# hasindu2008/cornetto

Measured on AMD Instinct MI355X. Metric: Gbases/s scanned (telowin+sdust+boringbits), higher is better.
Workload: dtype u8/u16 integer

## Files before the change

### cornetto_amd/__init__.py

```python
import ctypes as C
import os

import numpy as np

__all__ = ["lib", "Accel", "AccelError", "HIT_DT", "WIN_DT", "IVL_DT", "TELROW_DT", "khash_str_order", "panel_boring", "REG_DT", "REGREC_DT", "build",
           "LIB_PATH", "CLI_PATH"]

HERE = os.path.dirname(os.path.abspath(__file__))
DEV_LIB_PATH = os.path.join(HERE, "libcornetto_hip_dev.so")
LIB_PATH = os.environ.get("CORNETTO_LIB") or os.path.join(HERE, "libcornetto_hip.so")
CLI_PATH = os.path.join(HERE, "cornetto")

HIT_DT = np.dtype([("ctg", "<i4"), ("strand", "<i4"), ("start", "<i4"), ("end", "<i4")])
WIN_DT = np.dtype([("ctg", "<i4"), ("start", "<i4"), ("end", "<i4"), ("car", "<i4")])
IVL_DT = np.dtype([("ctg", "<i4"), ("start", "<i4"), ("finish", "<i4")])
TELROW_DT = np.dtype([("ctg", "<i4"), ("start", "<i4"), ("end", "<i4"), ("matched", "<i4")])
FQREC_DT = np.dtype([("head", "<i8"), ("seq", "<i8"), ("qual", "<i8"), ("len", "<i4"), ("name_len", "<i4"),
                     ("comment_len", "<i4"), ("keep", "<i4")])
EMITREC_DT = np.dtype([("ctg", "<i4"), ("rc", "<i4"), ("head", "<i8"), ("head_len", "<i8")])
FAREC_DT = np.dtype([("head", "<i8"), ("len", "<i8"), ("name_len", "<i4"), ("pad", "<i4")])
REG_DT = np.dtype([("st", "<i4"), ("end", "<i4"), ("depth", "<i4"), ("mq_depth", "<i4")])
REGREC_DT = np.dtype([("ctg", "<i4"), ("st", "<i4"), ("end", "<i4"), ("depth", "<i4"), ("mq_depth", "<i4")])
REGPK_DT = np.dtype([("st", "<i4"), ("depth", "<u2"), ("mq_depth", "<u2")])

# ... 342 lines not shown

    def telofind(self, asm, motif=b"TTAGGG"):
        p, n = C.c_void_p(), C.c_int64()
        self._chk(self.L.cornetto_telofind(self.h, asm.ptr, motif, C.byref(p), C.byref(n)))
        return _take(self.L, p, n.value, HIT_DT)

    def telowin_threshold(self, thr, identity):
        return self.L.cornetto_telowin_threshold(thr, identity)

    def telowin(self, hits, ctg_len, thr_adj):
        hits = np.ascontiguousarray(hits, dtype=HIT_DT)
        ctg_len = np.ascontiguousarray(ctg_len, dtype=np.int32)
        p, n = C.c_void_p(), C.c_int64()
        self._chk(self.L.cornetto_telowin(self.h, hits.ctypes.data, hits.size, ctg_len.ctypes.data, ctg_len.size,
                                          thr_adj, C.byref(p), C.byref(n)))
        return _take(self.L, p, n.value, WIN_DT)

    def telo_scan(self, asm, motif, thr_adj, want_hits=True):
        ph, nh, pw, nw = C.c_void_p(), C.c_int64(), C.c_void_p(), C.c_int64()
        self._chk(self.L.cornetto_telo_scan(self.h, asm.ptr, motif, thr_adj,
                                            C.byref(ph) if want_hits else None, C.byref(nh) if want_hits else None,
                                            C.byref(pw), C.byref(nw)))
        hits = _take(self.L, ph, nh.value, HIT_DT) if want_hits else None
        return hits, _take(self.L, pw, nw.value, WIN_DT)

    def telo_ends(self, asm, motif, thr_adj, merge_dist=100, ends=50000):
        p, n = C.c_void_p(), C.c_int64()
        self._chk(self.L.cornetto_telo_ends(self.h, asm.ptr, motif, thr_adj, merge_dist, ends, C.byref(p), C.byref(n)))
        return _take(self.L, p, n.value, IVL_DT)

    def sdust(self, asm, T=20, W=64):
        p, n = C.c_void_p(), C.c_int64()
        self._chk(self.L.cornetto_sdust_asm(self.h, asm.ptr, T, W, C.byref(p), C.byref(n)))
        return _take(self.L, p, n.value, IVL_DT)

    def sdust_begin(self, asm, T=20, W=64):
        self._chk(self.L.cornetto_sdust_asm_begin(self.h, asm.ptr, T, W))

    def sdust_end(self, asm, T=20, W=64):
        p, n = C.c_void_p(), C.c_int64()
        self._chk(self.L.cornetto_sdust_asm_end(self.h, asm.ptr, T, W, C.byref(p), C.byref(n)))
        return _take(self.L, p, n.value, IVL_DT)

    def sdust_stats(self, asm, T=20, W=64):
        self.L.cornetto_accel_sdust_stats(self.h, 1, None, 0)
        try:
            self.sdust(asm, T, W)
        finally:
            out = np.zeros(256, dtype=np.uint64)
            n = self.L.cornetto_accel_sdust_stats(self.h, 0, out.ctypes.data, 256)
        s = [int(x) for x in out[:n]]
        waves = s[254]
        if n > 207 and s[206]:
            return {"kernel": "sd_sift", "chunks": s[255], "tiles_of_64_bases": s[206], "positions_ct_above_T10": s[203], "after_L1": s[204], "after_L2": s[205],
                    "resolve_steps": s[200], "resolve_window_reads": s[201], "dp_tiles": s[208], "passes_with_candidates": s[202], "base_by_base_steps_of_chunks_with_other_bytes": s[207],
                    "window_reads_behind_a_gap_of": {"2": s[209], "3-4": s[210], "5-8": s[211]} if n > 211 else None}
        if not waves or not s[2]:
            return None
        hist = []
        for b in range(32):
            w = s[16 + 4 * b]
            if w:
                hist.append({"ms": [b * 0.5, b * 0.5 + 0.5], "waves": w, "jobs": s[18 + 4 * b], "find_perfect": s[19 + 4 * b], "find_perfect_with_candidates": s[17 + 4 * b]})
        return {"waves": waves, "chunks": s[255], "chunks_sampled_low_complexity": s[7], "wave_steps": s[2], "find_perfect_calls": s[3],
                "find_perfect_with_candidates": s[10], "plain_groups": s[4], "wave_ms_avg": round(s[5] / waves / 1e5, 3), "wave_ms_max": round(s[6] / 1e5, 3),
                "queue_fetch_rounds_per_wave": round(s[11] / waves, 1), "wave_time_histogram": hist}

    def cov_select_merged(self, cov, lo, hi, low_mq, edge_len, min_ctg_len, boring, merge_dist=1000, min_len=30000):
        p, n = C.c_void_p(), C.c_int64()
        self._chk(self.L.cornetto_cov_select_merged(self.h, cov.ptr, lo, hi, low_mq, edge_len, min_ctg_len, 1 if boring else 0, merge_dist, min_len,
                                                    C.byref(p), C.byref(n)))
        return _take(self.L, p, n.value, IVL_DT)

    def ivl_merge(self, ivls, dist):
        ivls = np.ascontiguousarray(ivls, dtype=IVL_DT)
        p, n = C.c_void_p(), C.c_int64()
        self._chk(self.L.cornetto_ivl_merge(self.h, ivls.ctypes.data, len(ivls), dist, C.byref(p), C.byref(n)))
        return _take(self.L, p, n.value, IVL_DT)

    def telobreaks(self, ctg_len, sd, tel):
        ctg_len = np.ascontiguousarray(ctg_len, dtype=np.int32)
        sd = np.ascontiguousarray(sd, dtype=IVL_DT)
        tel = np.ascontiguousarray(tel, dtype=TELROW_DT)
        p, n = C.c_void_p(), C.c_int64()
        self._chk(self.L.cornetto_telobreaks(self.h, ctg_len.ctypes.data, len(ctg_len), sd.ctypes.data, len(sd), tel.ctypes.data, len(tel),
                                             C.byref(p), C.byref(n)))
        return _take(self.L, p, n.value, IVL_DT)

    def cov_upload(self, depths, mqs):
        d = [np.ascontiguousarray(x, dtype=np.uint16) for x in depths]
        q = [np.ascontiguousarray(x, dtype=np.uint16) for x in mqs]
        n = len(d)
        pd = (C.c_void_p * max(n, 1))(*[a.ctypes.data for a in d])
        pq = (C.c_void_p * max(n, 1))(*[a.ctypes.data for a in q])
        lens = np.array([a.size for a in d], dtype=np.int32)
        out = C.c_void_p()
        self._chk(self.L.cornetto_cov_upload(self.h, pd, pq, lens.ctypes.data, n, C.byref(out)))
        return _Resident(self, out, self.L.cornetto_cov_free, lens)

    def cov_wrap(self, d_depth, d_mq, offsets, lens):
        offsets = np.ascontiguousarray(offsets, dtype=np.int64)
        lens = np.ascontiguousarray(lens, dtype=np.int32)
        out = C.c_void_p()
        self._chk(self.L.cornetto_cov_wrap(self.h, d_depth, d_mq, offsets.ctypes.data, lens.ctypes.data, len(lens), C.byref(out)))
        return _Resident(self, out, self.L.cornetto_cov_free, lens)

    def cov_shard(self, src_acc, cov, ctgs):
# ... 181 lines not shown
```

### cornetto_amd/csrc/sdust.hip

```cpp
#include <algorithm>
#include <type_traits>
#include <ctime>
#include <sched.h>

#include "common.hpp"
#include "scan.hpp"
#include "tiles.hpp"
#include "ivlmerge.hpp"

namespace {

__device__ __forceinline__ int nt4_code(uint32_t c);
struct SdArgs;
struct SdChunk;
template <bool LEAN = false>
__device__ int sd_find_start(const SdArgs &A, const SdChunk ch, const uint8_t *seq);

struct SdChunk {
    int32_t ctg, start, end;
};
struct SdChunkFill {
    SdChunk *out;
    const int32_t *len;
    int32_t chunk;
// ... 1554 lines not shown
        unsigned long long *d_tot = (unsigned long long *)cn_ws(h, WS_SD_STATS, 2048 + 64 * 64);
        unsigned long long *p_tot = (unsigned long long *)cn_pin(h, PIN_SMALL, 2048);
        if (!d_cnt || !d_tot || !p_tot) return cn_fail(h, CORNETTO_E_NOMEM, "sdust: workspace allocation failed");
        uint32_t *d_off = d_cnt + nc;
        stamp("small workspaces");
        const bool env_stats = CN_DEV_INT("CORNETTO_SDUST_STATS", 0) != 0;
        const bool want_stats = env_stats || h->sd_stats != 0;
        size_t cap = (size_t)std::max<int64_t>(16, chunk / 32);
        cap = (size_t)CN_DEV_INT("CORNETTO_SDUST_CAP", (int)cap);
        if (h->dev[WS_SD_OUT].bytes / (nc * sizeof(uint2)) > cap) cap = h->dev[WS_SD_OUT].bytes / (nc * sizeof(uint2));
        unsigned long long tot = 0;
        uint2 *d_out = nullptr;
        const int64_t est_key = key * 131 + T * 1031 + W;
        const bool one_go = w64_path && sift_on && !want_stats && a->sd_est_key == est_key && a->sd_est_rows >= 0 && CN_DEV_INT("CORNETTO_SDUST_FUSED", 1);
        if (phase == 1 && !one_go)
            return CORNETTO_OK;
        for (int attempt = 0; attempt < 4; ++attempt) {
            d_out = (uint2 *)cn_ws(h, WS_SD_OUT, nc * cap * sizeof(uint2));
            if (!d_out) return cn_fail(h, CORNETTO_E_NOMEM, "sdust: workspace allocation of %zu bytes failed", nc * cap * sizeof(uint2));
            CN_HIP(h, hipMemsetAsync(d_tot, 0, 2048 + 64 * 64, h->stream));
            uint32_t *d_slots = (uint32_t *)cn_ws(h, WS_SD_OFF, (size_t)(std::max<int64_t>(sd_waves, 1) + SD_WPB) * 64 * 64 * sizeof(uint32_t));
            if (!d_slots) return cn_fail(h, CORNETTO_E_NOMEM, "sdust: workspace allocation failed");
            stamp("row + slot workspaces");
            const bool use_w64 = w64_path;
            SdArgs A{a->d_bases, a->d_off, a->d_len, d_chunks, (int32_t)nc, T, W, d_out, d_cnt, (uint32_t)cap,
                     want_stats ? d_tot + 2 : nullptr, reinterpret_cast<uint32_t *>(d_tot + 1), d_slots, nullptr,
                     reinterpret_cast<uint32_t *>(d_tot + 8), nullptr, 0, CN_DEV_INT("CORNETTO_SDUST_RUNON", 1), (int32_t)chunk, a->d_wtab, a->d_wtab_base, reinterpret_cast<uint32_t *>(d_tot + 1) + 1};
            unsigned nb = (unsigned)((nc + 63) / 64);
            bool sift_walk_pending = false;
            bool dense_pending = false;
            struct DenseJoin {
                cornetto_accel_t *h;
                bool *pending;
                ~DenseJoin() { if (*pending && h->stream2) (void)hipStreamSynchronize(h->stream2); }
            } dense_join{h, &dense_pending};
            if (use_w64 && sift_on) {
                CN_HIP(h, hipMemsetAsync(d_cnt, 0, nc * 4, h->stream));
                const uint32_t reg_cap = (uint32_t)(chunk + 128);
                const uint32_t lds_wave = sift_lds_bytes(reg_cap);
                int lmin = 1;
                while (5 * (lmin + 1) <= T && lmin < 16) ++lmin;
                const bool walk_known = a->d_sd_walk && a->sd_walk_key == key;
                const size_t walk_words = 2 + 4 * nc + 2;
                if (!walk_known) {
                    if (a->d_sd_walk) { (void)hipFree(a->d_sd_walk); a->d_sd_walk = nullptr; }
                    a->sd_walk_key = -1;
                    if (cn_obj_malloc(h, (void **)&a->d_sd_walk, walk_words * 4) != hipSuccess) return cn_fail(h, CORNETTO_E_NOMEM, "sdust: device allocation failed");
                    CN_HIP(h, hipMemsetAsync(a->d_sd_walk, 0, (2 + 2 * nc) * 4, h->stream));
                }
                uint32_t *d_wflag = a->d_sd_walk + 2 + nc, *d_wrank = d_wflag + nc, *d_worder = d_wrank + nc;
                SiftArgs S{a->d_bases, a->d_off, a->d_len, d_chunks, (int32_t)nc, T, W, lds_wave, reg_cap,
                           walk_known ? d_worder : nullptr, walk_known ? nullptr : a->d_sd_walk, walk_known ? nullptr : d_wflag,
                           reinterpret_cast<uint32_t *>(d_tot + 256), T / 10 + 1, lmin, CN_DEV_INT("CORNETTO_SIFT_ABL", 0),
                           std::min(65, std::max(1, CN_DEV_INT("CORNETTO_SIFT_DP", 24))), std::min(65, std::max(1, CN_DEV_INT("CORNETTO_SIFT_L2SKIP", 48)))};
                sift_walk_pending = !walk_known;
                SdArgs R = A;
                R.stats = want_stats ? d_tot + 200 : nullptr;
                const bool cap_default = reg_cap == SIFT_CAP_DEFAULT && !CN_DEV_INT("CORNETTO_SIFT_GENERIC", 0) && !CN_DEV_INT("CORNETTO_SIFT_ABL", 0);
                if (h->sift_per_cu == 0 || h->sift_per_cu_default != (cap_default ? 1 : 0)) {
                    int per_cu = 0;
                    const hipError_t oe = cap_default ? hipOccupancyMaxActiveBlocksPerMultiprocessor(&per_cu, sd_sift<false, SIFT_CAP_DEFAULT>, 64 * SIFT_WPB, lds_wave * SIFT_WPB)
                                                      : hipOccupancyMaxActiveBlocksPerMultiprocessor(&per_cu, sd_sift<false>, 64 * SIFT_WPB, lds_wave * SIFT_WPB);
                    if (oe != hipSuccess || per_cu < 1) per_cu = 8;
                    h->sift_per_cu = per_cu;
                    h->sift_per_cu_default = cap_default ? 1 : 0;
                }
                const int per_cu_all = std::max(1, std::min<int>(h->sift_per_cu, (int)(163840 / ((lds_wave * SIFT_WPB + 1279) / 1280 * 1280))));
                const bool free_now = __atomic_load_n(&h->boost, __ATOMIC_ACQUIRE) != 0;
                const size_t cus_n = (size_t)std::max(h->sd_cus, 1);
                const size_t slots_all = (size_t)per_cu_all * cus_n;
                const size_t slots = free_now ? slots_all : std::max<size_t>(cus_n, slots_all * (size_t)h->share / 100);
                const size_t all_blocks = (nc + SIFT_WPB - 1) / SIFT_WPB;
                const unsigned nbk = (unsigned)std::min<size_t>(all_blocks, (size_t)CN_DEV_INT("CORNETTO_SIFT_BLOCKS", (int)slots));
                const unsigned extra = (unsigned)std::min<size_t>(all_blocks > nbk ? all_blocks - nbk : 0, slots_all > slots ? slots_all - slots : 0);
                const bool may_help = phase == 0 && extra > 0 && !want_stats && h->share < CN_DEV_INT("CORNETTO_SDUST_HELP_BELOW", 70);
                if (may_help) {
                    if (!h->stream2) {
                        int pr_least = 0, pr_greatest = 0;
                        (void)hipDeviceGetStreamPriorityRange(&pr_least, &pr_greatest);
                        CN_HIP(h, hipStreamCreateWithPriority(&h->stream2, hipStreamNonBlocking, pr_greatest));
                        CN_HIP(h, hipEventCreateWithFlags(&h->ev2, hipEventDisableTiming));
                        CN_HIP(h, hipEventCreateWithFlags(&h->ev1, hipEventDisableTiming));
                    }
                    if (!h->ev3) CN_HIP(h, hipEventCreateWithFlags(&h->ev3, hipEventDisableTiming));
                    CN_HIP(h, hipEventRecord(h->ev1, h->stream));
                }
                stamp("set up");
                if (want_stats) CN_LAUNCH(h, "sdust_kernel", sd_sift<true><<<dim3(nbk), dim3(64 * SIFT_WPB), lds_wave * SIFT_WPB, h->stream>>>(S, R));
                else if (cap_default) CN_LAUNCH(h, "sdust_kernel", sd_sift<false, SIFT_CAP_DEFAULT><<<dim3(nbk), dim3(64 * SIFT_WPB), lds_wave * SIFT_WPB, h->stream>>>(S, R));
                else CN_LAUNCH(h, "sdust_kernel", sd_sift<false><<<dim3(nbk), dim3(64 * SIFT_WPB), lds_wave * SIFT_WPB, h->stream>>>(S, R));
                __atomic_fetch_add(&h->launch_seq, 1ull, __ATOMIC_RELEASE);
                if (may_help) {
                    CN_HIP(h, hipEventRecord(h->ev3, h->stream));
                    bool helped = false;
                    while (hipEventQuery(h->ev3) == hipErrorNotReady) {
                        if (!helped && __atomic_load_n(&h->boost, __ATOMIC_ACQUIRE) != 0) {
                            CN_HIP(h, hipStreamWaitEvent(h->stream2, h->ev1, 0));
                            if (cap_default) sd_sift<false, SIFT_CAP_DEFAULT><<<dim3(extra), dim3(64 * SIFT_WPB), lds_wave * SIFT_WPB, h->stream2>>>(S, R);
                            else sd_sift<false><<<dim3(extra), dim3(64 * SIFT_WPB), lds_wave * SIFT_WPB, h->stream2>>>(S, R);
                            dense_pending = true;
                            CN_HIP(h, hipGetLastError());
                            CN_HIP(h, hipEventRecord(h->ev2, h->stream2));
                            helped = true;
                        }
                        sched_yield();
                    }
                    if (helped) CN_HIP(h, hipStreamWaitEvent(h->stream, h->ev2, 0));
// ... 118 lines not shown
                dense_pending = false;
            }
            CN_TRY(cnscan::exclusive_u32(h, "sdust_scan", d_cnt, (int64_t)nc, 1, d_off, d_tot));
            if (one_go) {
                size_t n_cap = (size_t)(a->sd_est_rows + a->sd_est_rows / 8 + 4096);
                if (CN_DEV_INT("CORNETTO_SDUST_EST_FORCE", 0) > 0) n_cap = (size_t)CN_DEV_INT("CORNETTO_SDUST_EST_FORCE", 0);
                const size_t m_cap = (size_t)(a->sd_est_out + a->sd_est_out / 16 + 1024);
                uint8_t *ws = (uint8_t *)cn_ws(h, WS_SD_DST, 2 * n_cap * sizeof(cornetto_ivl_t) + cnivl::ws_bytes(n_cap));
                cornetto_ivl_t *of = (cornetto_ivl_t *)cn_result_alloc(std::max<size_t>(m_cap * sizeof(cornetto_ivl_t), (size_t)1 << 20));
                if (ws && of && n_cap < 0x7fffffffull) {
                    cornetto_ivl_t *d_dst = (cornetto_ivl_t *)(ws + cnivl::ws_bytes(n_cap)), *d_st = d_dst + n_cap;
                    const unsigned nbg = (unsigned)((nc + 255) / 256);
                    CN_LAUNCH(h, "sdust_gather", sdust_gather<<<dim3(nbg), dim3(256), 0, h->stream>>>(d_out, d_cnt, d_off, (uint32_t)cap, d_chunks, (int32_t)nc, d_dst, (uint32_t)n_cap));
                    CN_HIP(h, hipMemsetAsync(d_tot + 9, 0xFF, 8, h->stream));
                    int rcf = cnivl::merge_fused(h, "sdust_stitch", d_dst, d_tot, (int64_t)n_cap, 0, d_st, d_tot + 9);
                    if (rcf != CORNETTO_OK) { cornetto_free(of); return rcf; }
                    stamp("tail queued");
                    if (hipMemcpyAsync(of, d_st, m_cap * sizeof(cornetto_ivl_t), hipMemcpyDeviceToHost, h->stream) != hipSuccess ||
                        hipMemcpyAsync(p_tot, d_tot, 128, hipMemcpyDeviceToHost, h->stream) != hipSuccess) {
                        (void)hipStreamSynchronize(h->stream);
                        cornetto_free(of);
                        return cn_fail(h, CORNETTO_E_HIP, "sdust: stitch / copy back failed");
                    }
                    if (phase == 1) {
                        h->sd_pend.state = 1; h->sd_pend.a = a; h->sd_pend.T = T; h->sd_pend.W = W; h->sd_pend.of = of;
                        h->sd_pend.m_cap = m_cap; h->sd_pend.n_cap = n_cap; h->sd_pend.cap = cap; h->sd_pend.key = key; h->sd_pend.walk_pending = sift_walk_pending;
                        return CORNETTO_OK;
                    }
                    const int fin = sd_one_go_finish(h, a, of, p_tot, cap, n_cap, m_cap, key, sift_walk_pending, ivls, n_ivls);
                    if (fin <= 0) {
                        if (fin == 0) stamp("results on the host (one go)");
                        return fin;
                    }
                } else if (of) {
                    cornetto_free(of);
                }
            }
            stamp("main kernel queued");
            CN_HIP(h, hipMemcpyAsync(p_tot, d_tot, want_stats ? 2048 : 128, hipMemcpyDeviceToHost, h->stream));
            CN_HIP(h, hipStreamSynchronize(h->stream));
            stamp("main kernel done");
            if (want_stats) {
                memcpy(h->sd_last, p_tot, 2048);
                if (a->sd_flagged >= 0) h->sd_last[7] = (unsigned long long)a->sd_flagged;
                h->sd_last[254] = nb;
                h->sd_last[255] = nc;
            }
            if (env_stats)
                for (int b = 0; b < 32; ++b)
                    if (p_tot[16 + 4 * b])
                        fprintf(stderr, "[sdust stats]   waves that ran %4.1f-%4.1f ms: %6llu, job fetches %llu, find_perfect calls %llu (%llu with candidates)\n", b * 0.5, b * 0.5 + 0.5,
                                p_tot[16 + 4 * b], p_tot[18 + 4 * b], p_tot[19 + 4 * b], p_tot[17 + 4 * b]);
            if (env_stats && sift_on)
                fprintf(stderr, "[sdust stats] sift: tiles %llu, positions with ct > T/10 %llu, after L1 %llu, after L2 %llu; resolve: steps %llu, window reads %llu (behind a gap of 2 / 3-4 / 5-8: %llu / %llu / %llu), dp tiles %llu; passes with candidates %llu; base-by-base steps of chunks with other bytes %llu\n",
                        p_tot[206], p_tot[203], p_tot[204], p_tot[205], p_tot[200], p_tot[201], p_tot[209], p_tot[210], p_tot[211], p_tot[208], p_tot[202], p_tot[207]);
            if (env_stats)
                fprintf(stderr, "[sdust stats] flagged low-complexity %llu; chunks %zu waves %u wave-steps %llu find_perfect calls %llu (%llu with candidates) plain groups %llu; wave time avg %.1f us max %.1f us; queue: %.1f fetch rounds and %.1f us per wave\n", p_tot[7], nc, nb,
                        p_tot[2], p_tot[3], p_tot[10], p_tot[4], nb ? (double)p_tot[5] / nb / 100.0 : 0.0, (double)p_tot[6] / 100.0, nb ? (double)p_tot[11] / nb : 0.0, nb ? (double)p_tot[12] / nb / 100.0 : 0.0);
            const uint32_t ovf = (uint32_t)(p_tot[1] & 0xFFFFFFFFull);
            const bool need_wtab = (p_tot[1] >> 32) != 0;
            if (need_wtab) {
                if (a->d_wtab) return cn_fail(h, CORNETTO_E_HIP, "sdust: word-count table requested twice");
                std::vector<int64_t> base(a->n + 1, 0);
                for (int32_t c = 0; c < a->n; ++c) base[c + 1] = base[c] + a->len[c] / SD_WBLK + 2;
                a->n_wblocks = base[a->n];
                uint32_t *d_wcnt = nullptr;
                if (hipMalloc((void **)&a->d_wtab, ((size_t)a->n_wblocks + 1) * 4) != hipSuccess ||
                    hipMalloc((void **)&a->d_wtab_base, ((size_t)a->n + 1) * 8) != hipSuccess ||
                    hipMalloc((void **)&d_wcnt, ((size_t)a->n_wblocks + 1) * 4) != hipSuccess)
                    return cn_fail(h, CORNETTO_E_NOMEM, "sdust: word-count table allocation failed");
                CN_HIP(h, hipMemcpyAsync(a->d_wtab_base, base.data(), ((size_t)a->n + 1) * 8, hipMemcpyHostToDevice, h->stream));
                const unsigned nbw = (unsigned)((a->n_wblocks + 255) / 256);
                CN_LAUNCH(h, "sd_wordcount", sd_wordcount<<<dim3(nbw), dim3(256), 0, h->stream>>>(a->d_bases, a->d_off, a->d_len, a->d_wtab_base, a->n,
                                                                                         a->n_wblocks, d_wcnt));
                int rc = cnscan::exclusive_u32(h, "sd_wordscan", d_wcnt, a->n_wblocks, 1, a->d_wtab, nullptr);
                hipError_t e = hipStreamSynchronize(h->stream);
                (void)hipFree(d_wcnt);
                if (rc != CORNETTO_OK) return rc;
                if (e != hipSuccess) return cn_fail(h, CORNETTO_E_HIP, "sdust: word-count table build failed");
                continue;
            }
            if (sift_walk_pending && !need_wtab) a->sd_walk_key = key;
            if (ovf <= cap) {
                tot = p_tot[0];
                break;
            }
            if (attempt >= 2) return cn_fail(h, CORNETTO_E_HIP, "sdust: a chunk produced %u intervals after resizing to %zu", ovf, cap);
            cap = ovf;
        }
        if (tot > 0x7fffffffull) return cn_fail(h, CORNETTO_E_UNSUPPORTED, "sdust: %llu intervals", tot);
        o = (cornetto_ivl_t *)cn_result_alloc((tot ? tot : 1) * sizeof(cornetto_ivl_t));
        if (!o) return cn_fail(h, CORNETTO_E_NOMEM, "sdust: host allocation failed");
        stamp("result buffer");
        if (tot > 0) {
            const size_t n = (size_t)tot;
            uint8_t *ws = (uint8_t *)cn_ws(h, WS_SD_DST, 2 * n * sizeof(cornetto_ivl_t) + cnivl::ws_bytes(n));
            if (!ws) { cornetto_free(o); return cn_fail(h, CORNETTO_E_NOMEM, "sdust: workspace allocation failed"); }
            cornetto_ivl_t *d_dst = (cornetto_ivl_t *)(ws + cnivl::ws_bytes(n)), *d_st = d_dst + n;
            const unsigned nbg = (unsigned)((nc + 255) / 256);
            CN_LAUNCH(h, "sdust_gather", sdust_gather<<<dim3(nbg), dim3(256), 0, h->stream>>>(d_out, d_cnt, d_off, (uint32_t)cap, d_chunks, (int32_t)nc, d_dst));
            CN_TRY(cnivl::merge(h, "sdust_stitch", d_dst, (int64_t)n, 0, ws, d_st, d_tot + 9));
            stamp("gather+stitch queued");
            if (trace) { (void)hipStreamSynchronize(h->stream); stamp("gather+stitch done (trace only)"); }
            if (hipMemcpyAsync(o, d_st, n * sizeof(cornetto_ivl_t), hipMemcpyDeviceToHost, h->stream) != hipSuccess ||
                hipMemcpyAsync(p_tot, d_tot + 9, 8, hipMemcpyDeviceToHost, h->stream) != hipSuccess ||
                hipStreamSynchronize(h->stream) != hipSuccess) {
                cornetto_free(o);
// ... 148 lines not shown
```

### cornetto_amd/csrc/sdust_sift.hpp

```cpp
#pragma once

struct SiftArgs {
    const uint8_t *bases;
    const int64_t *ctg_off;
    const int32_t *ctg_len;
    const SdChunk *chunks;
    int32_t n_chunks;
    int32_t T, W;
    uint32_t lds_per_wave;
    uint32_t reg_cap;
    const uint32_t *order;
    uint32_t *walk_out;
    uint32_t *iswalk_out;
    uint32_t *counter;
    int32_t thr, lmin;
    int32_t abl;
    int32_t dp_min;
    int32_t l2_skip;
};

#ifndef SIFT_WPB
#define SIFT_WPB 1
#endif
constexpr int SIFT_NCTR = 64;
constexpr int SIFT_PAD = 16;
#ifndef SIFT_K
#define SIFT_K 16
#endif
constexpr int SIFT_LS = SIFT_K - 1;
constexpr int SIFT_FIXED = 1024 + 512;
__host__ __device__ constexpr uint32_t sift_lds_bytes(uint32_t cap) { return (SIFT_FIXED + cap / 4 + 2 * (SIFT_PAD + cap) + 16 + 15) / 16 * 16; }


__device__ __forceinline__ uint32_t sd_codes4(uint32_t word)
{
    const uint32_t y = word & 0xDFDFDFDFu, idx = y & 0x07070707u;
    const uint32_t code = __builtin_amdgcn_perm(0x02000003u, 0x01000000u, idx);
    const uint32_t d = y ^ __builtin_amdgcn_perm(0x47FFFF54u, 0x43FF41FFu, idx);
    const uint32_t nz = ((d & 0x7F7F7F7Fu) + 0x7F7F7F7Fu) | d;
    return code | ((nz >> 5) & 0x04040404u);
}
__device__ __forceinline__ uint32_t sd_words4(uint32_t cn, uint32_t pcn)
{
    const uint32_t y1 = __builtin_amdgcn_alignbyte(cn, pcn, 3);
    const uint32_t y2 = __builtin_amdgcn_alignbyte(cn, pcn, 2);
    const uint32_t t = (cn & 0x03030303u) | ((y1 & 0x03030303u) << 2) | ((y2 & 0x03030303u) << 4);
    return t | (((cn | y1 | y2) & 0x04040404u) << 4);
}

__device__ __forceinline__ int sd_mbcnt64(unsigned long long m)
{
    return (int)__builtin_amdgcn_mbcnt_hi((uint32_t)(m >> 32), __builtin_amdgcn_mbcnt_lo((uint32_t)m, 0u));
}
__device__ __forceinline__ int sd_dpp_shr1(int old, int src, bool zero_fill)
{
    return zero_fill ? __builtin_amdgcn_update_dpp(0, src, 0x138, 0xF, 0xF, true) : __builtin_amdgcn_update_dpp(old, src, 0x138, 0xF, 0xF, false);
}

__device__ const uint32_t sd_recip_tab[64] = {0x0u, 0x0u, 0x80000000u, 0x55555556u, 0x40000000u, 0x33333334u, 0x2AAAAAABu, 0x24924925u, 0x20000000u, 0x1C71C71Du, 0x1999999Au, 0x1745D175u, 0x15555556u, 0x13B13B14u, 0x12492493u, 0x11111112u, 0x10000000u, 0xF0F0F10u, 0xE38E38Fu, 0xD79435Fu, 0xCCCCCCDu, 0xC30C30Du, 0xBA2E8BBu, 0xB21642Du, 0xAAAAAABu, 0xA3D70A4u, 0x9D89D8Au, 0x97B425Fu, 0x924924Au, 0x8D3DCB1u, 0x8888889u, 0x8421085u, 0x8000000u, 0x7C1F07Du, 0x7878788u, 0x7507508u, 0x71C71C8u, 0x6EB3E46u, 0x6BCA1B0u, 0x6906907u, 0x6666667u, 0x63E7064u, 0x6186187u, 0x5F417D1u, 0x5D1745Eu, 0x5B05B06u, 0x590B217u, 0x572620Bu, 0x5555556u, 0x539782Au, 0x51EB852u, 0x5050506u, 0x4EC4EC5u, 0x4D4873Fu, 0x4BDA130u, 0x4A7904Bu, 0x4924925u, 0x47DC120u, 0x469EE59u, 0x456C798u, 0x4444445u, 0x4325C54u, 0x4210843u, 0x4104105u};

__device__ __forceinline__ uint32_t sd_scan_max_dpp(uint32_t x)
{
    asm volatile("s_nop 1\n\t"
                 "v_max_u32_dpp %0, %0, %0 row_shr:1 row_mask:0xf bank_mask:0xf\n\ts_nop 1\n\t"
                 "v_max_u32_dpp %0, %0, %0 row_shr:2 row_mask:0xf bank_mask:0xf\n\ts_nop 1\n\t"
                 "v_max_u32_dpp %0, %0, %0 row_shr:4 row_mask:0xf bank_mask:0xf\n\ts_nop 1\n\t"
                 "v_max_u32_dpp %0, %0, %0 row_shr:8 row_mask:0xf bank_mask:0xf\n\ts_nop 1\n\t"
                 "v_max_u32_dpp %0, %0, %0 row_bcast:15 row_mask:0xa bank_mask:0xf\n\ts_nop 1\n\t"
                 "v_max_u32_dpp %0, %0, %0 row_bcast:31 row_mask:0xc bank_mask:0xf\n\ts_nop 1"
                 : "+v"(x));
    return x;
}

__device__ __forceinline__ int sd_wave_find_start(const SdChunk ch, const uint8_t *seq, int W, int lane)
{
    if (ch.start <= 0) return 0;
    const int y = ch.start - 2 * W;
    if (y <= 2) return 0;
    int need = W - 2;
    for (int tile = (y - 1) >> 6, it = 0; tile >= 0 && it < 64; --tile, ++it) {
        const int p = tile * 64 + lane;
        const bool isb = p < y && nt4_code(seq[p]) < 4;
        const unsigned long long b = sd_ballot(isb);
        need -= __popcll(b & (b << 1) & (b << 2));
        if (need <= 0 || tile == 0) return tile * 64;
    }
    return -2;
}

#ifndef SIFT_CHUNK_DEFAULT
#define SIFT_CHUNK_DEFAULT 1792
#endif
constexpr uint32_t SIFT_CAP_DEFAULT = SIFT_CHUNK_DEFAULT + 128;
template <bool STATS, uint32_t CAP = 0>
__global__ __launch_bounds__(64 * SIFT_WPB) __attribute__((amdgpu_waves_per_eu(CAP ? 7 : 6))) void sd_sift(SiftArgs A, SdArgs O)
{
    extern __shared__ __attribute__((aligned(16))) uint8_t sift_lds[];
    const int lane = threadIdx.x & 63;
    const int wave = SIFT_WPB == 1 ? 0 : __builtin_amdgcn_readfirstlane((int)(threadIdx.x >> 6));
    uint8_t *const L = sift_lds + (size_t)wave * (CAP ? sift_lds_bytes(CAP) : A.lds_per_wave);
    uint32_t *const tab = reinterpret_cast<uint32_t *>(L);
    uint16_t *const tl = reinterpret_cast<uint16_t *>(L + 1024);
    uint16_t *const tl2 = tl + 128;
    uint32_t *const sb = reinterpret_cast<uint32_t *>(L + SIFT_FIXED);
    const uint32_t cap = CAP ? CAP : A.reg_cap;
#ifdef CN_DEV
    const int abl = CAP ? 0 : A.abl;
#else
    constexpr int abl = 0;
#endif
    constexpr int STAGE_ROUNDS = CAP ? (int)((CAP + 1023) / 1024) : 4;
    uint32_t *const cb = sb + (cap >> 5);
    uint4 *const col = reinterpret_cast<uint4 *>(tab);
    uint8_t *const wc = L + SIFT_FIXED + cap / 4 + 2 * SIFT_PAD;
    const int T = A.T, W = A.W, CAPW = W - 2;

    const int lo = lane - (CAPW - 1);
    const unsigned long long below = lane ? ~0ull >> (64 - lane) : 0ull;
    const unsigned long long mc = lo > 0 ? below & (~0ull << lo) : below;
    const unsigned long long mp = lo < 0 ? ~0ull << (64 + lo) : 0ull;
    const uint32_t m_a = (uint32_t)mc, m_d = (uint32_t)(mp >> 32), m_m = lane < 32 ? (uint32_t)mp : (uint32_t)(mc >> 32);
    const uint32_t mybit = 1u << (lane & 31);
    uint32_t *const mine0 = tab + (lane < 32 ? 0 : 192), *const mine1 = tab + (lane < 32 ? 64 : 128);
    uint32_t *const tab_mine = mine0;
    const uint32_t *const mid1 = tab + (lane < 32 ? 0 : 128);
    const int thr = A.thr, lmin = A.lmin;
    const int LS = CAPW - 1 < SIFT_LS ? CAPW - 1 : SIFT_LS;
    const bool long_ok = CAPW - 1 > LS;
    unsigned long long st_steps = 0, st_jumps = 0, st_cand = 0, st_trig = 0, st_l1 = 0, st_l2 = 0, st_walk = 0, st_tiles = 0, st_dp = 0, st_g2 = 0, st_g4 = 0, st_g8 = 0;

    struct Meta {
        SdChunk ch;
        int len;
        const uint8_t *seq;
    };
    struct Data {
        uint4 q[2];
        uint32_t pw[2];
    };
    auto meta = [&](int kk) {
        Meta m;
        m.ch = A.chunks[kk];
        m.len = A.ctg_len[m.ch.ctg];
        m.seq = A.bases + A.ctg_off[m.ch.ctg];
        return m;
    };
    auto fetch = [&](const Meta &m) {
        Data d;
        const int rb = m.ch.start - (m.ch.start > 0 ? 128 : 0), rlen = m.ch.end - rb;
#pragma unroll
        for (int it = 0; it < 2; ++it) {
            const int b16 = lane * 16 + it * 1024;
            d.q[it] = make_uint4(0, 0, 0, 0);
            if (b16 < rlen) d.q[it] = *reinterpret_cast<const uint4 *>(m.seq + rb + b16);
        }
        uint32_t first = 0;
        if (rb > 0) first = *reinterpret_cast<const uint32_t *>(m.seq + rb - 4);
        d.pw[0] = (uint32_t)__builtin_amdgcn_update_dpp((int)first, (int)d.q[0].w, 0x138, 0xF, 0xF, false);
        d.pw[1] = (uint32_t)__builtin_amdgcn_update_dpp(rdlane((int)d.q[0].w, 63), (int)d.q[1].w, 0x138, 0xF, 0xF, false);
        return d;
    };

  auto process = [&](const int k, const Meta &M, const Data &D) {
    const SdChunk ch = M.ch;
    const int len = M.len;
    const uint8_t *seq = M.seq;
    const int halo = ch.start > 0 ? 128 : 0;
    const int rb = ch.start - halo;
    const int rlen = ch.end - rb;
    const int ntile = (rlen + 63) >> 6;
    const bool islast = ch.end == len;
    const int rec_from = ch.start;

    tab[lane] = 0;
    tab[64 + lane] = 0;
    tab[128 + lane] = 0;
    tab[192 + lane] = 0;
    for (int i = lane; i < (int)(cap >> 4); i += 64) sb[i] = 0;
    if (lane < SIFT_PAD) reinterpret_cast<uint16_t *>(wc)[lane - SIFT_PAD] = halo ? 0xFF40 : 0x0040;
    bool bad = false;
    bool general = rb <= 0 || rb + ((rlen + 15) & ~15) > len || (abl & 32);
// ... 137 lines not shown

    if (unclean) {
        const int Tl = T * lane;
        const uint32_t m_recip = sd_recip_tab[lane];
        if (A.walk_out && lane == 0) {
            A.iswalk_out[k] = 1u;
            A.walk_out[2 + atomicAdd(&A.walk_out[0], 1u)] = (uint32_t)k;
        }
        int u = sd_wave_find_start(ch, seq, W, lane);
        if (u == -2) u = __builtin_amdgcn_readfirstlane(sd_find_start<true>(O, ch, seq));
        if (u < 0) return;
        const int stop = islast ? len + 1 : ch.end;
        int l = 0, size = 0, cv = 4, ctile = -1;
        unsigned t = 0;
        for (int i = u; i < stop; ++i) {
            if ((i >> 6) != ctile) {
                ctile = i >> 6;
                const int p = ctile * 64 + lane;
                cv = p < len ? nt4_code(seq[p]) : 4;
            }
            const int b = rdlane(cv, i & 63);
            if (STATS) ++st_walk;
            if (b < 4) {
                ++l;
                t = (t << 2 | (unsigned)b) & 63u;
                if (l >= 3) {
                    const int start = (l - W > 0 ? l - W : 0) + (i + 1 - l);
                    const bool full = size >= CAPW;
                    const bool moves = l > W;
                    if (full && moves) {
                        const uint32_t so = (uint32_t)rdlane(slot, CAPW - 1);
                        if (so) {
                            const int s = sv0 - (CAPW - 1);
                            emit(s, s + (int)(so >> 24) + 3, i);
                        }
                    }
                    size = full ? CAPW : size + 1;
                    push_word((int)t, size - 1, !full || moves);
                    sv0 = start + size - 1;
                    pass(size - 1, Tl, m_recip);
                }
            } else {
                emit_slots(0, i);
                slot = 0;
                l = 0;
                t = 0;
            }
        }
        finish();
        return;
    }

    typedef __attribute__((address_space(3))) uint32_t lds_u32;
    int ntl = 0, ntl2 = 0;
#ifdef SIFT_L2_ADAPT
    int l2_hot = 0, l2_skipped = 0;
#endif
    auto run_l2 = [&](int nb) {
        const bool on = lane < nb;
        const int o = on ? (int)tl2[lane] : 0;
        bool keep = on;
        if (LS == SIFT_LS) {
            const uint32_t at = (uint32_t)(uintptr_t)(lds_u32 *)wc + 2u * (uint32_t)o - 2u * (uint32_t)(SIFT_K - 1);
            const lds_u32 *const pa = (const lds_u32 *)(uintptr_t)(at & ~3u);
            const uint32_t sh = at & 3u;
            uint32_t k80, ksel1, ksel2, ksel3, kw, kc;
            asm volatile("s_mov_b32 %0, 0x3f3f3f3f\n\ts_mov_b32 %1, 0x01010101\n\ts_mov_b32 %2, 0x02020202\n\ts_mov_b32 %3, 0x03030303\n\t"
                         "s_mov_b32 %4, 0x06040200\n\ts_mov_b32 %5, 0x07050301"
                         : "=s"(k80), "=s"(ksel1), "=s"(ksel2), "=s"(ksel3), "=s"(kw), "=s"(kc));
            uint32_t tt = (uint32_t)T;
            asm volatile("" : "+s"(tt));
            uint32_t Q[4];
#pragma unroll
            for (int q = 0; q < 4; ++q) {
                const uint32_t d0 = pa[2 * q], d1 = pa[2 * q + 1], d2 = pa[2 * q + 2];
                Q[q] = __builtin_amdgcn_perm(__builtin_amdgcn_alignbyte(d2, d1, sh), __builtin_amdgcn_alignbyte(d1, d0, sh), kc);
            }
            uint32_t S = 0;
            unsigned long long pos_m = ~0ull;
#pragma unroll
            for (int a = 0; a < SIFT_K; ++a) {
                const int idx = SIFT_K - 1 - a;
                switch (idx & 3) {
                case 0: asm("v_add_u32_sdwa %0, %1, %0 dst_sel:DWORD dst_unused:UNUSED_PAD src0_sel:BYTE_0 src1_sel:DWORD" : "+v"(S) : "v"(Q[idx >> 2])); break;
                case 1: asm("v_add_u32_sdwa %0, %1, %0 dst_sel:DWORD dst_unused:UNUSED_PAD src0_sel:BYTE_1 src1_sel:DWORD" : "+v"(S) : "v"(Q[idx >> 2])); break;
                case 2: asm("v_add_u32_sdwa %0, %1, %0 dst_sel:DWORD dst_unused:UNUSED_PAD src0_sel:BYTE_2 src1_sel:DWORD" : "+v"(S) : "v"(Q[idx >> 2])); break;
                default: asm("v_add_u32_sdwa %0, %1, %0 dst_sel:DWORD dst_unused:UNUSED_PAD src0_sel:BYTE_3 src1_sel:DWORD" : "+v"(S) : "v"(Q[idx >> 2])); break;
                }
                const uint32_t th = (tt * (uint32_t)(a + 1)) / 10u;
                unsigned long long ok = __builtin_amdgcn_ballot_w64(S > th);
                asm volatile("" : "+s"(ok), "+v"(S));
                pos_m &= ok;
            }
            uint32_t at2 = at & ~3u;
            asm volatile("" : "+v"(at2), "+s"(pos_m));
            const lds_u32 *const pb = (const lds_u32 *)(uintptr_t)at2;
            uint32_t P[4];
#pragma unroll
            for (int q = 0; q < 4; ++q) {
                const uint32_t d0 = pb[2 * q], d1 = pb[2 * q + 1], d2 = pb[2 * q + 2];
                P[q] = __builtin_amdgcn_perm(__builtin_amdgcn_alignbyte(d2, d1, sh), __builtin_amdgcn_alignbyte(d1, d0, sh), kw);
            }
            const uint32_t seen = (P[0] | P[1] | P[2] | P[3]) & 0xC0C0C0C0u;
            uint32_t ne = 0;
            unsigned long long sc_m = 0ull;
#pragma unroll
            for (int a = 1; a < SIFT_K; ++a) {
                const int idx = SIFT_K - 1 - a, qi = idx >> 2, bj = idx & 3;
                const uint32_t rep = __builtin_amdgcn_perm(P[qi], P[qi], bj == 0 ? 0u : bj == 1 ? ksel1 : bj == 2 ? ksel2 : ksel3);
#pragma unroll
                for (int q = qi; q < 4; ++q) {
                    if (q == qi && bj == 3) continue;
                    const uint32_t m = q == qi ? 0x40404040u << (8 * (bj + 1)) : 0x40404040u;
                    const uint32_t u = (P[q] ^ rep) + k80;
                    ne += (uint32_t)__builtin_popcount(u & m);
                }
                const int lim = a * (a + 1) / 2 - (int)((tt * (uint32_t)a) / 10u);
                unsigned long long hit = __builtin_amdgcn_ballot_w64((int)ne < lim);
                asm volatile("" : "+s"(hit), "+v"(ne), "+v"(P[0]), "+v"(P[1]), "+v"(P[2]), "+v"(P[3]));
                sc_m |= hit;
            }
            const bool sc = (sc_m >> lane) & 1ull, pos = (pos_m >> lane) & 1ull;
            keep = on && (seen != 0u || sc || (pos && long_ok));
        }
        if (STATS) st_l2 += (unsigned long long)__popcll(sd_ballot(keep));
#ifdef SIFT_L2_ADAPT
        if (nb == 64) {
            const int kept = __popcll(sd_ballot(keep));
            l2_hot = kept >= SIFT_L2_ADAPT ? (l2_hot < 2 ? l2_hot + 1 : 2) : 0;
            l2_skipped = 0;
        }
#endif
        if (keep) (void)__hip_atomic_fetch_or(&sb[o >> 5], 1u << (o & 31), __ATOMIC_RELAXED, __HIP_MEMORY_SCOPE_WORKGROUP);
    };
    auto run_l1 = [&](int nb) {
        const bool on = lane < nb;
        const int o = on ? (int)tl[lane] : 0;
        const uint8_t *const p = wc + 2 * o;
        int d = 0, dmin = 0x7fffffff;
        if (lmin == 4) {
            uint32_t tt = (uint32_t)T;
            asm volatile("" : "+s"(tt));
            const uint32_t c0 = p[1], c1 = p[-1], c2 = p[-3], c3 = p[-5];
            const uint32_t s1 = c0 + c1, s2 = s1 + c2, s3 = s2 + c3;
            dmin = ((c0 > tt / 10u) & (s1 > (2u * tt) / 10u) & (s2 > (3u * tt) / 10u) & (s3 > (4u * tt) / 10u)) ? 1 : 0;
        } else {
            for (int j = 0; j < lmin; ++j) {
                d += 10 * (int)p[1 - 2 * j] - T;
                dmin = d < dmin ? d : dmin;
            }
        }
        const bool ok = on && dmin > 0;
        const unsigned long long m = sd_ballot(ok);
#ifdef SIFT_L2_ADAPT
        const bool hot = l2_hot >= 2 && __popcll(m) >= 16;
        if (hot && ++l2_skipped >= 12) l2_hot = 1;
        if (__popcll(m) >= A.l2_skip || hot) {
#else
        if (__popcll(m) >= A.l2_skip) {
#endif
            if (STATS) st_l1 += (unsigned long long)__popcll(m);
            if (STATS) st_l2 += (unsigned long long)__popcll(m);
            if (ok) (void)__hip_atomic_fetch_or(&sb[o >> 5], 1u << (o & 31), __ATOMIC_RELAXED, __HIP_MEMORY_SCOPE_WORKGROUP);
        } else if (m) {
            if (STATS) st_l1 += (unsigned long long)__popcll(m);
            if (ok) tl2[ntl2 + sd_mbcnt64(m)] = (uint16_t)o;
            ntl2 += __popcll(m);
            SD_LDS_ORDER();
            if (ntl2 >= 64) {
                run_l2(64);
                const uint16_t mv = tl2[64 + lane];
                SD_LDS_ORDER();
                tl2[lane] = mv;
                ntl2 -= 64;
                SD_LDS_ORDER();
            }
        }
    };

    uint8_t *pq = wc + 2 * lane;
    const uint32_t tab_a = (uint32_t)(uintptr_t)(lds_u32 *)tab, mine0_a = (uint32_t)(uintptr_t)(lds_u32 *)mine0, mine1_a = (uint32_t)(uintptr_t)(lds_u32 *)mine1,
                   mid1_a = (uint32_t)(uintptr_t)(lds_u32 *)mid1;
    auto lds_at = [](uint32_t wi, uint32_t base) __attribute__((always_inline)) {
        uint32_t a;
        asm("v_lshl_add_u32 %0, %1, 2, %2" : "=v"(a) : "v"(wi), "v"(base));
        return (lds_u32 *)(uintptr_t)a;
    };
    uint32_t wv_ahead = pq[0];
    auto tile = [&](auto par_c, auto general_c, auto only_c, const int q) __attribute__((always_inline)) {
        constexpr int PAR = decltype(par_c)::value;
        constexpr bool GENERAL = decltype(general_c)::value, TABLE_ONLY = decltype(only_c)::value;
        constexpr int A_AT = PAR ? 64 : 0, D_AT = PAR ? 192 : 128, M_AT = PAR ? 0 : 64;
        constexpr int Z0 = PAR ? 0 : 64, Z1 = PAR ? 192 : 128;
        constexpr bool CHECK = GENERAL || TABLE_ONLY;
        const uint32_t wv = wv_ahead;
        wv_ahead = pq[128];
        asm("" : "+v"(wv_ahead));
        const bool valid = !CHECK || (wv < 64u && q * 64 + lane < rlen);
        const uint32_t wi = CHECK ? wv & 63u : wv;
        lds_u32 *const t_mine = lds_at(wi, PAR ? mine1_a : mine0_a), *const t_all = lds_at(wi, tab_a), *const t_mid = lds_at(wi, mid1_a);
        if (valid) (void)__hip_atomic_fetch_or(t_mine, mybit, __ATOMIC_RELAXED, __HIP_MEMORY_SCOPE_WORKGROUP);
        SD_LDS_ORDER();
        const uint32_t e_a = t_all[A_AT], e_m = t_mid[M_AT], e_d = t_all[D_AT];
        SD_LDS_ORDER();
        tab[Z0 + lane] = 0;
        tab[Z1 + lane] = 0;
        uint32_t ctu = (uint32_t)__popc(e_a & m_a);
        asm("v_bcnt_u32_b32 %0, %1, %0" : "+v"(ctu) : "v"(e_m & m_m));
        asm("v_bcnt_u32_b32 %0, %1, %0" : "+v"(ctu) : "v"(e_d & m_d));
        const int ct = (int)ctu;
        pq[1] = (uint8_t)(TABLE_ONLY ? 255 : (valid ? ct : 0));
        pq += 128;
        if (!TABLE_ONLY) {
            const bool trig = valid && ct >= thr;
            const unsigned long long m = sd_ballot(trig);
            if (m) {
                if (STATS) st_trig += (unsigned long long)__popcll(m);
                int idx;
                asm("v_cndmask_b32_e64 %0, 64, %1, %2" : "=v"(idx) : "v"(sd_mbcnt64(m)), "s"(m));
                (tl + ntl)[idx] = (uint16_t)(q * 64 + lane);
                ntl += __popcll(m);
                SD_LDS_ORDER();
                if (ntl >= 64) {
                    if (!(abl & 2)) run_l1(64);
                    const uint16_t mv = tl[64 + lane];
                    SD_LDS_ORDER();
                    tl[lane] = mv;
                    ntl -= 64;
                    SD_LDS_ORDER();
                }
            }
        }
    };
    if (!(abl & 4)) {
        using P0 = std::integral_constant<int, 0>;
        using P1 = std::integral_constant<int, 1>;
        int q = 0;
        if (halo) tile(P0{}, std::false_type{}, std::true_type{}, q++);
        else tile(P0{}, std::true_type{}, std::false_type{}, q++);
        for (; q + 1 < ntile - 1; q += 2) {
            tile(P1{}, std::false_type{}, std::false_type{}, q);
            tile(P0{}, std::false_type{}, std::false_type{}, q + 1);
        }
        if (q < ntile - 1) { tile(P1{}, std::false_type{}, std::false_type{}, q); ++q; }
        if (q < ntile) {
            if (q & 1) tile(P1{}, std::true_type{}, std::false_type{}, q);
            else tile(P0{}, std::true_type{}, std::false_type{}, q);
        }
    }
    SD_LDS_ORDER();
    if (ntl > 0 && !(abl & 2)) run_l1(ntl);
    if (ntl2 > 0) run_l2(ntl2);
    if (abl & 1) { finish(); return; }
    SD_LDS_ORDER();

    const int s_lo = ch.start > 0 ? ch.start - W : -0x40000000, s_hi = islast ? 0x7fffffff : ch.end - W;
    int lane_r = lane;
    asm volatile("" : "+v"(lane_r));
    const int Tl = T * lane_r;
    const uint32_t m_recip = sd_recip_tab[lane_r];
    auto mark64 = [&](int o, int nbits) {
        const uint32_t d = (uint32_t)o >> 5, b = (uint32_t)o & 31u;
        const unsigned long long mk = nbits >= 64 ? ~0ull : (1ull << nbits) - 1ull;
        const unsigned long long lo64 = mk << b;
        const uint32_t w1 = (uint32_t)(lo64 >> 32), w2 = b ? (uint32_t)(mk >> (64u - b)) : 0u;
        (void)__hip_atomic_fetch_or(&cb[d], (uint32_t)lo64, __ATOMIC_RELAXED, __HIP_MEMORY_SCOPE_WORKGROUP);
        if (w1) (void)__hip_atomic_fetch_or(&cb[d + 1], w1, __ATOMIC_RELAXED, __HIP_MEMORY_SCOPE_WORKGROUP);
        if (w2) (void)__hip_atomic_fetch_or(&cb[d + 2], w2, __ATOMIC_RELAXED, __HIP_MEMORY_SCOPE_WORKGROUP);
    };
    auto mark = [&](int s, int nbits) {
        if (s < s_lo || s >= s_hi) return;
        if (nbits > 64) {
            mark64(s - rb, 64);
            mark64(s - rb + 64, nbits - 64);
        } else {
            mark64(s - rb, nbits);
        }
    };
    auto pass_m = [&](int amax) {
        const unsigned long long cm = sd_ballot(__mul24(r, 10) > Tl) & ~(~1ull << amax) & ~1ull;
        if (cm) {
            const bool cand = (cm >> lane) & 1ull;
            if (STATS) ++st_cand;
            uint32_t key_c = 0u;
            if (cand) key_c = lane == 1 ? ((uint32_t)r & 0x7FFu) << 13 : __umulhi(((uint32_t)r & 0x7FFu) << 13, m_recip);
            const uint32_t key_e = (uint32_t)slot;
            const uint32_t xs = sd_scan_max_dpp(key_e > key_c ? key_e : key_c);
            const uint32_t sk = (uint32_t)__builtin_amdgcn_update_dpp(0, (int)xs, 0x138, 0xF, 0xF, true);
            const uint32_t km = sk > key_e ? sk : key_e;
            if (cand && key_c >= km) {
                slot = (int)key_c;
                mark(sv0 - lane, lane + 3);
            }
        }
    };

    unsigned long long sw = 0;
    if (lane < ntile) sw = (unsigned long long)sb[2 * lane] | (unsigned long long)sb[2 * lane + 1] << 32;
    if (halo) {
        if (lane == 0) sw = 0;
        if (lane == 1) sw &= ~0ull << (66 - W);
    } else if (lane == 0) {
        sw &= ~3ull;
    }
    tab[lane] = 0;
// ... 253 lines not shown
```

Before: 499.3.

## Merge sift L1/L2 filters into one deep test with shorter lookback

Replaces the two-stage candidate filter (L1 prefix test, then a compacted L2 queue with a quadratic pairwise-equality test) with a single pass. This pass folds the L1 check into the deep prefix-sum loop and uses a cheaper linear repeat-count test against the last base. It removes the second LDS queue, its compaction and syncs, and the l2_skip heuristic. It also shrinks the lookback K from 16 to 12 and frees LDS per wave. The cheaper short-period test may pass more candidates to the resolve stage, and the deep test now runs on every L1 batch instead of only sparse ones.

```diff
diff --git a/cornetto_amd/__init__.py b/cornetto_amd/__init__.py
--- a/cornetto_amd/__init__.py
+++ b/cornetto_amd/__init__.py
@@ -418,7 +418,7 @@
         s = [int(x) for x in out[:n]]
         waves = s[254]
         if n > 207 and s[206]:
-            return {"kernel": "sd_sift", "chunks": s[255], "tiles_of_64_bases": s[206], "positions_ct_above_T10": s[203], "after_L1": s[204], "after_L2": s[205],
+            return {"kernel": "sd_sift", "chunks": s[255], "tiles_of_64_bases": s[206], "positions_ct_above_T10": s[203], "after_L1": s[204], "after_deep_test": s[205],
                     "resolve_steps": s[200], "resolve_window_reads": s[201], "dp_tiles": s[208], "passes_with_candidates": s[202], "base_by_base_steps_of_chunks_with_other_bytes": s[207],
                     "window_reads_behind_a_gap_of": {"2": s[209], "3-4": s[210], "5-8": s[211]} if n > 211 else None}
         if not waves or not s[2]:
diff --git a/cornetto_amd/csrc/sdust.hip b/cornetto_amd/csrc/sdust.hip
--- a/cornetto_amd/csrc/sdust.hip
+++ b/cornetto_amd/csrc/sdust.hip
@@ -1630,7 +1630,7 @@
                 SiftArgs S{a->d_bases, a->d_off, a->d_len, d_chunks, (int32_t)nc, T, W, lds_wave, reg_cap,
                            walk_known ? d_worder : nullptr, walk_known ? nullptr : a->d_sd_walk, walk_known ? nullptr : d_wflag,
                            reinterpret_cast<uint32_t *>(d_tot + 256), T / 10 + 1, lmin, CN_DEV_INT("CORNETTO_SIFT_ABL", 0),
-                           std::min(65, std::max(1, CN_DEV_INT("CORNETTO_SIFT_DP", 24))), std::min(65, std::max(1, CN_DEV_INT("CORNETTO_SIFT_L2SKIP", 48)))};
+                           std::min(65, std::max(1, CN_DEV_INT("CORNETTO_SIFT_DP", 24)))};
                 sift_walk_pending = !walk_known;
                 SdArgs R = A;
                 R.stats = want_stats ? d_tot + 200 : nullptr;
@@ -1855,7 +1855,7 @@
                         fprintf(stderr, "[sdust stats]   waves that ran %4.1f-%4.1f ms: %6llu, job fetches %llu, find_perfect calls %llu (%llu with candidates)\n", b * 0.5, b * 0.5 + 0.5,
                                 p_tot[16 + 4 * b], p_tot[18 + 4 * b], p_tot[19 + 4 * b], p_tot[17 + 4 * b]);
             if (env_stats && sift_on)
-                fprintf(stderr, "[sdust stats] sift: tiles %llu, positions with ct > T/10 %llu, after L1 %llu, after L2 %llu; resolve: steps %llu, window reads %llu (behind a gap of 2 / 3-4 / 5-8: %llu / %llu / %llu), dp tiles %llu; passes with candidates %llu; base-by-base steps of chunks with other bytes %llu\n",
+                fprintf(stderr, "[sdust stats] sift: tiles %llu, positions with ct > T/10 %llu, after L1 %llu, after the deep test %llu; resolve: steps %llu, window reads %llu (behind a gap of 2 / 3-4 / 5-8: %llu / %llu / %llu), dp tiles %llu; passes with candidates %llu; base-by-base steps of chunks with other bytes %llu\n",
                         p_tot[206], p_tot[203], p_tot[204], p_tot[205], p_tot[200], p_tot[201], p_tot[209], p_tot[210], p_tot[211], p_tot[208], p_tot[202], p_tot[207]);
             if (env_stats)
                 fprintf(stderr, "[sdust stats] flagged low-complexity %llu; chunks %zu waves %u wave-steps %llu find_perfect calls %llu (%llu with candidates) plain groups %llu; wave time avg %.1f us max %.1f us; queue: %.1f fetch rounds and %.1f us per wave\n", p_tot[7], nc, nb,
diff --git a/cornetto_amd/csrc/sdust_sift.hpp b/cornetto_amd/csrc/sdust_sift.hpp
--- a/cornetto_amd/csrc/sdust_sift.hpp
+++ b/cornetto_amd/csrc/sdust_sift.hpp
@@ -16,7 +16,6 @@
     int32_t thr, lmin;
     int32_t abl;
     int32_t dp_min;
-    int32_t l2_skip;
 };
 
 #ifndef SIFT_WPB
@@ -25,10 +24,10 @@
 constexpr int SIFT_NCTR = 64;
 constexpr int SIFT_PAD = 16;
 #ifndef SIFT_K
-#define SIFT_K 16
+#define SIFT_K 12
 #endif
-constexpr int SIFT_LS = SIFT_K - 1;
-constexpr int SIFT_FIXED = 1024 + 512;
+static_assert(SIFT_K % 4 == 0 && SIFT_K >= 4 && SIFT_K <= SIFT_PAD, "SIFT_K: 4, 8, 12 or 16");
+constexpr int SIFT_FIXED = 1024 + 256;
 __host__ __device__ constexpr uint32_t sift_lds_bytes(uint32_t cap) { return (SIFT_FIXED + cap / 4 + 2 * (SIFT_PAD + cap) + 16 + 15) / 16 * 16; }
 
 
@@ -101,7 +100,6 @@
     uint8_t *const L = sift_lds + (size_t)wave * (CAP ? sift_lds_bytes(CAP) : A.lds_per_wave);
     uint32_t *const tab = reinterpret_cast<uint32_t *>(L);
     uint16_t *const tl = reinterpret_cast<uint16_t *>(L + 1024);
-    uint16_t *const tl2 = tl + 128;
     uint32_t *const sb = reinterpret_cast<uint32_t *>(L + SIFT_FIXED);
     const uint32_t cap = CAP ? CAP : A.reg_cap;
 #ifdef CN_DEV
@@ -125,8 +123,6 @@
     uint32_t *const tab_mine = mine0;
     const uint32_t *const mid1 = tab + (lane < 32 ? 0 : 128);
     const int thr = A.thr, lmin = A.lmin;
-    const int LS = CAPW - 1 < SIFT_LS ? CAPW - 1 : SIFT_LS;
-    const bool long_ok = CAPW - 1 > LS;
     unsigned long long st_steps = 0, st_jumps = 0, st_cand = 0, st_trig = 0, st_l1 = 0, st_l2 = 0, st_walk = 0, st_tiles = 0, st_dp = 0, st_g2 = 0, st_g4 = 0, st_g8 = 0;
 
     struct Meta {
@@ -370,29 +366,44 @@
     }
 
     typedef __attribute__((address_space(3))) uint32_t lds_u32;
-    int ntl = 0, ntl2 = 0;
-#ifdef SIFT_L2_ADAPT
-    int l2_hot = 0, l2_skipped = 0;
-#endif
-    auto run_l2 = [&](int nb) {
+    int ntl = 0;
+    const bool deep = CAPW >= SIFT_K;
+    const bool long_ok = CAPW - 1 >= SIFT_K;
+    auto run_l1 = [&](int nb) {
         const bool on = lane < nb;
-        const int o = on ? (int)tl2[lane] : 0;
-        bool keep = on;
-        if (LS == SIFT_LS) {
+        const int o = on ? (int)tl[lane] : 0;
+        unsigned long long l1_m = ~0ull;
+        if (!deep || lmin > SIFT_K) {
+            const uint8_t *const p = wc + 2 * o;
+            int d = 0, dmin = 0x7fffffff;
+            for (int j = 0; j < lmin; ++j) {
+                d += 10 * (int)p[1 - 2 * j] - T;
+                dmin = d < dmin ? d : dmin;
+            }
+            l1_m = sd_ballot(dmin > 0);
+        }
+        bool keep = on && ((l1_m >> lane) & 1ull);
+        if (deep) {
             const uint32_t at = (uint32_t)(uintptr_t)(lds_u32 *)wc + 2u * (uint32_t)o - 2u * (uint32_t)(SIFT_K - 1);
             const lds_u32 *const pa = (const lds_u32 *)(uintptr_t)(at & ~3u);
             const uint32_t sh = at & 3u;
-            uint32_t k80, ksel1, ksel2, ksel3, kw, kc;
-            asm volatile("s_mov_b32 %0, 0x3f3f3f3f\n\ts_mov_b32 %1, 0x01010101\n\ts_mov_b32 %2, 0x02020202\n\ts_mov_b32 %3, 0x03030303\n\t"
-                         "s_mov_b32 %4, 0x06040200\n\ts_mov_b32 %5, 0x07050301"
-                         : "=s"(k80), "=s"(ksel1), "=s"(ksel2), "=s"(ksel3), "=s"(kw), "=s"(kc));
+            uint32_t k3f, ksel3, kw, kc;
+            asm volatile("s_mov_b32 %0, 0x3f3f3f3f\n\ts_mov_b32 %1, 0x03030303\n\ts_mov_b32 %2, 0x06040200\n\ts_mov_b32 %3, 0x07050301"
+                         : "=s"(k3f), "=s"(ksel3), "=s"(kw), "=s"(kc));
             uint32_t tt = (uint32_t)T;
             asm volatile("" : "+s"(tt));
-            uint32_t Q[4];
+            constexpr int NQ = SIFT_K / 4;
+            uint32_t Q[NQ], P[NQ];
+            {
+                uint32_t dw[2 * NQ + 1];
 #pragma unroll
-            for (int q = 0; q < 4; ++q) {
-                const uint32_t d0 = pa[2 * q], d1 = pa[2 * q + 1], d2 = pa[2 * q + 2];
-                Q[q] = __builtin_amdgcn_perm(__builtin_amdgcn_alignbyte(d2, d1, sh), __builtin_amdgcn_alignbyte(d1, d0, sh), kc);
+                for (int i = 0; i < 2 * NQ + 1; ++i) dw[i] = pa[i];
+#pragma unroll
+                for (int q = 0; q < NQ; ++q) {
+                    const uint32_t a0 = __builtin_amdgcn_alignbyte(dw[2 * q + 1], dw[2 * q], sh), a1 = __builtin_amdgcn_alignbyte(dw[2 * q + 2], dw[2 * q + 1], sh);
+                    Q[q] = __builtin_amdgcn_perm(a1, a0, kc);
+                    P[q] = __builtin_amdgcn_perm(a1, a0, kw);
+                }
             }
             uint32_t S = 0;
             unsigned long long pos_m = ~0ull;
@@ -409,91 +420,23 @@
                 unsigned long long ok = __builtin_amdgcn_ballot_w64(S > th);
                 asm volatile("" : "+s"(ok), "+v"(S));
                 pos_m &= ok;
-            }
-            uint32_t at2 = at & ~3u;
-            asm volatile("" : "+v"(at2), "+s"(pos_m));
-            const lds_u32 *const pb = (const lds_u32 *)(uintptr_t)at2;
-            uint32_t P[4];
+                if (a + 1 == lmin) l1_m = pos_m;
+            }
+            const uint32_t rep = __builtin_amdgcn_perm(P[NQ - 1], P[NQ - 1], ksel3);
+            uint32_t ne = 0, seen = 0;
 #pragma unroll
-            for (int q = 0; q < 4; ++q) {
-                const uint32_t d0 = pb[2 * q], d1 = pb[2 * q + 1], d2 = pb[2 * q + 2];
-                P[q] = __builtin_amdgcn_perm(__builtin_amdgcn_alignbyte(d2, d1, sh), __builtin_amdgcn_alignbyte(d1, d0, sh), kw);
-            }
-            const uint32_t seen = (P[0] | P[1] | P[2] | P[3]) & 0xC0C0C0C0u;
-            uint32_t ne = 0;
-            unsigned long long sc_m = 0ull;
-#pragma unroll
-            for (int a = 1; a < SIFT_K; ++a) {
-                const int idx = SIFT_K - 1 - a, qi = idx >> 2, bj = idx & 3;
-                const uint32_t rep = __builtin_amdgcn_perm(P[qi], P[qi], bj == 0 ? 0u : bj == 1 ? ksel1 : bj == 2 ? ksel2 : ksel3);
-#pragma unroll
-                for (int q = qi; q < 4; ++q) {
-                    if (q == qi && bj == 3) continue;
-                    const uint32_t m = q == qi ? 0x40404040u << (8 * (bj + 1)) : 0x40404040u;
-                    const uint32_t u = (P[q] ^ rep) + k80;
-                    ne += (uint32_t)__builtin_popcount(u & m);
-                }
-                const int lim = a * (a + 1) / 2 - (int)((tt * (uint32_t)a) / 10u);
-                unsigned long long hit = __builtin_amdgcn_ballot_w64((int)ne < lim);
-                asm volatile("" : "+s"(hit), "+v"(ne), "+v"(P[0]), "+v"(P[1]), "+v"(P[2]), "+v"(P[3]));
-                sc_m |= hit;
-            }
-            const bool sc = (sc_m >> lane) & 1ull, pos = (pos_m >> lane) & 1ull;
-            keep = on && (seen != 0u || sc || (pos && long_ok));
-        }
+            for (int q = 0; q < NQ; ++q) {
+                const uint32_t u = (P[q] ^ rep) + k3f;
+                ne += (uint32_t)__builtin_popcount(u & 0x40404040u);
+                seen |= P[q];
+            }
+            const bool l1 = (l1_m >> lane) & 1ull, pos = (pos_m >> lane) & 1ull;
+            const bool shortc = (int)ne <= SIFT_K - 1 - thr;
+            keep = on && l1 && ((seen & 0x40404040u) != 0u || shortc || (pos && long_ok));
+        }
+        if (STATS) st_l1 += (unsigned long long)__popcll(l1_m & (nb >= 64 ? ~0ull : (1ull << nb) - 1ull));
         if (STATS) st_l2 += (unsigned long long)__popcll(sd_ballot(keep));
-#ifdef SIFT_L2_ADAPT
-        if (nb == 64) {
-            const int kept = __popcll(sd_ballot(keep));
-            l2_hot = kept >= SIFT_L2_ADAPT ? (l2_hot < 2 ? l2_hot + 1 : 2) : 0;
-            l2_skipped = 0;
-        }
-#endif
         if (keep) (void)__hip_atomic_fetch_or(&sb[o >> 5], 1u << (o & 31), __ATOMIC_RELAXED, __HIP_MEMORY_SCOPE_WORKGROUP);
-    };
-    auto run_l1 = [&](int nb) {
-        const bool on = lane < nb;
-        const int o = on ? (int)tl[lane] : 0;
-        const uint8_t *const p = wc + 2 * o;
-        int d = 0, dmin = 0x7fffffff;
-        if (lmin == 4) {
-            uint32_t tt = (uint32_t)T;
-            asm volatile("" : "+s"(tt));
-            const uint32_t c0 = p[1], c1 = p[-1], c2 = p[-3], c3 = p[-5];
-            const uint32_t s1 = c0 + c1, s2 = s1 + c2, s3 = s2 + c3;
-            dmin = ((c0 > tt / 10u) & (s1 > (2u * tt) / 10u) & (s2 > (3u * tt) / 10u) & (s3 > (4u * tt) / 10u)) ? 1 : 0;
-        } else {
-            for (int j = 0; j < lmin; ++j) {
-                d += 10 * (int)p[1 - 2 * j] - T;
-                dmin = d < dmin ? d : dmin;
-            }
-        }
-        const bool ok = on && dmin > 0;
-        const unsigned long long m = sd_ballot(ok);
-#ifdef SIFT_L2_ADAPT
-        const bool hot = l2_hot >= 2 && __popcll(m) >= 16;
-        if (hot && ++l2_skipped >= 12) l2_hot = 1;
-        if (__popcll(m) >= A.l2_skip || hot) {
-#else
-        if (__popcll(m) >= A.l2_skip) {
-#endif
-            if (STATS) st_l1 += (unsigned long long)__popcll(m);
-            if (STATS) st_l2 += (unsigned long long)__popcll(m);
-            if (ok) (void)__hip_atomic_fetch_or(&sb[o >> 5], 1u << (o & 31), __ATOMIC_RELAXED, __HIP_MEMORY_SCOPE_WORKGROUP);
-        } else if (m) {
-            if (STATS) st_l1 += (unsigned long long)__popcll(m);
-            if (ok) tl2[ntl2 + sd_mbcnt64(m)] = (uint16_t)o;
-            ntl2 += __popcll(m);
-            SD_LDS_ORDER();
-            if (ntl2 >= 64) {
-                run_l2(64);
-                const uint16_t mv = tl2[64 + lane];
-                SD_LDS_ORDER();
-                tl2[lane] = mv;
-                ntl2 -= 64;
-                SD_LDS_ORDER();
-            }
-        }
     };
 
     uint8_t *pq = wc + 2 * lane;
@@ -568,7 +511,6 @@
     }
     SD_LDS_ORDER();
     if (ntl > 0 && !(abl & 2)) run_l1(ntl);
-    if (ntl2 > 0) run_l2(ntl2);
     if (abl & 1) { finish(); return; }
     SD_LDS_ORDER();
 
```

After: 469.6. -5.9%, worse.
